# bi-graph/Emgraph

Measured on AMD Instinct MI355X. Metric: positive+negative triples scored/sec at k=200, eta=20; filtered ranks/sec, higher is better.
Workload: dtype f32; 1 GPU; C3: ComplEx k=200 (k_int=400) eta=20, synthetic |E|=1M |R|=1k, B=16384/GPU, NLL, SGD; B_per_gpu=16384, global_batch=16384, eta=20, k_int=400, k_int_per_gpu=400, n_ent=1000000, n_rel=1000, parallelism=single

## Files before the change

emgraph_amd/csrc/emg_score.hip:

```cpp
#include <math.h>
#include <string.h>

#include <atomic>

#include "emg_score_kernels.hpp"

namespace emg {

enum class Pass { Forward, Backward, Fused };

constexpr double kMallBytes = 256.0 * 1024 * 1024;
constexpr double kResidentBudget = 240e6;
static bool cache_policy_form(const GroupParams& P) {
    const int forced = sw_int(SW_CACHE_POLICY);
    if (forced == 0 || forced == 1) return forced == 1;
    const double n = (double)P.n_ent, row = 4.0 * (double)P.ld_ent;
    if (n < 2 || n * row <= kMallBytes) return false;
    const double N = (double)P.B * (2 + P.eta);
    const double l = log1p(-1.0 / n);
    const double distinct = n * -expm1(N * l), singles = N * exp((N - 1) * l);
    const double multi = distinct > singles ? distinct - singles : 0.0;
    const double contrib = 5.0 * (double)P.B + (P.fac.coef ? 0.0 : (N - singles));
    return (multi + contrib) * row <= kResidentBudget;
}

static std::atomic<int64_t> g_cache_policy_launches{0};

enum RidersGo : int32_t { RIDERS_NONE = 0, RIDERS_RIDE = 1, RIDERS_ALONE = 2 };
struct StepForm {
    Pass pass; int32_t model, n;
    int32_t W, shape;
    int32_t ip;
    bool wave_per_group, cache_policy, linked;
    int32_t riders;
    int32_t blocks;
};
static const int32_t kShape[8][2] = {{1, 16}, {1, 32}, {1, 64}, {2, 64}, {1, 64}, {2, 64}, {4, 64}, {8, 64}};
static int ladder(bool vec, int c, bool wave_per_group) {
    if (vec) return c <= 16 && !wave_per_group ? 0 : (c <= 32 && !wave_per_group ? 1 : (c <= kWaveChunks ? 2 : (c <= kMaxChunks ? 3 : -1)));
    return c <= 64 ? 4 : (c <= 128 ? 5 : (c <= 256 ? 6 : (c <= kColumnBlock ? 7 : -1)));
}

static int decide_step_form(Pass pass, int model, const GroupParams& P, bool have_riders, StepForm* out) {
    StepForm f{};
    f.pass = pass; f.model = model;
    const int n = f.n = step_columns(model, P.k_int);
    if (P.lr_hist && P.opt.opt == EMG_OPT_SGD) {
        EMG_REQUIRE(replay_rows(n, kMaxChunks, P.ld_ent, P.ent),
                    "emg_train_backward_ex: lr_hist needs 16-byte rows of at most %d chunks (per half for complex models)", kMaxChunks);
    } else if (P.lr_hist) {
        EMG_REQUIRE(replay_rows(n, kWaveChunks, P.ld_ent, P.ent) && aligned16(P.ent_state0) && aligned16(P.ent_state1) && !P.ctl,
                    "emg_train_backward_ex: lr_hist needs 16-byte rows of at most %d chunks (per half for complex models) and no device-side step record", kWaveChunks);
    }
    const bool cplx = (model == EMG_COMPLEX || model == EMG_HOLE);
    EMG_REQUIRE(model >= 0 && model <= EMG_HOLE, "unknown model id %d", model);
    EMG_REQUIRE(P.k_int > 0 && (!cplx || P.k_int % 2 == 0), "bad k_int %d for model %d", P.k_int, model);
    EMG_REQUIRE(P.ld_ent >= P.k_int && P.ld_rel >= P.k_int, "row stride smaller than k_int");
    EMG_REQUIRE(P.B >= 0 && P.eta >= 0, "negative sizes");
    if (P.B == 0) { *out = f; return EMG_OK; }
    EMG_REQUIRE(P.B * (int64_t)kThreads < ((int64_t)1 << 37), "batch too large");
    bool vec = (n % 4 == 0) && (P.ld_ent % 4 == 0) && (P.ld_rel % 4 == 0) && aligned16(P.ent) && aligned16(P.rel);
    if (pass != Pass::Forward) {
        vec = vec && (P.ldc % 4 == 0) && aligned16(P.contrib_ent) && aligned16(P.contrib_rel);
        if (P.single_ent)
            vec = vec && (!P.ent_state0 || aligned16(P.ent_state0)) && (!P.ent_state1 || aligned16(P.ent_state1));
    }
    f.W = vec ? 4 : 1;
    const bool sgd = P.opt.opt == EMG_OPT_SGD;
    if (pass != Pass::Forward && P.single_ent && sgd && P.opt.lp_lambda != 0.f && !vec)
        return fail(EMG_ENOSUP, "train backward: in-place updates fold an LP regulariser for 16-byte aligned rows only (k, or k per "
                                "half for complex models, a multiple of 4); pass single_ent = NULL");
    if (P.window && !(vec && pass == Pass::Fused && n / 4 <= kWaveChunks && P.single_ent && !sgd))
        return fail(EMG_ENOSUP, "train backward: inplace_window (a stateful optimizer's state rows travelling with the table rows) needs the "
                                "fused kernel on 16-byte aligned rows of at most %d chunks (per half for complex models)", kWaveChunks);
    if (pass == Pass::Forward || !P.single_ent) f.ip = IP_NONE;
    else if (sgd) f.ip = P.opt.lp_lambda == 0.f ? IP_SGD : (P.lr_hist ? IP_SGD_LP_LAG : IP_SGD_LP);
    else if (!P.window) f.ip = IP_STATE;
    else f.ip = P.lr_hist ? IP_WINDOW_LAG : ((P.opt.opt == EMG_OPT_ADAM || P.opt.opt == EMG_OPT_ADAM_LAZY) ? IP_WINDOW_2 : IP_WINDOW_1);
    f.riders = !have_riders ? RIDERS_NONE : ((pass == Pass::Fused && vec && n <= kColumnBlock) ? RIDERS_RIDE : RIDERS_ALONE);
    const int wide_env = sw_int(SW_WIDE_GROUPS);
    f.wave_per_group = f.ip >= IP_WINDOW_1 || (pass != Pass::Forward && (wide_env >= 0 ? wide_env != 0 : P.B <= 2048));
    f.blocks = 1; f.shape = ladder(vec, n / f.W, f.wave_per_group);
    if (f.shape < 0 && pass == Pass::Fused)
        return fail(EMG_ENOSUP, "fused score+loss+gradient: rows of k_int=%d are wider than the register-tiled kernel holds "
                                "(512 columns per half) — use emg_train_forward + emg_loss + emg_train_backward_ex(fused_loss = -1), "
                                "which splits wide rows into column blocks", P.k_int);
    if (f.shape < 0 && pass == Pass::Backward) {
        EMG_REQUIRE(model != EMG_TRANSE_L2 || (P.bw_scores_pos && (P.eta == 0 || P.bw_scores_neg)),
                    "train backward: TransE-L2 rows wider than 512 columns need bw_scores_pos / bw_scores_neg (the full norms)");
        f.blocks = (int32_t)cdiv(n, kColumnBlock);
        f.shape = ladder(vec, kColumnBlock / f.W, f.wave_per_group);
    }
    f.linked = pass == Pass::Fused && (P.link != EMG_LINK_LINEAR || P.edge_w);
    f.cache_policy = pass == Pass::Fused && f.shape == 2 && f.ip == IP_SGD && cache_policy_form(P);
    *out = f;
    return EMG_OK;
}

struct ShapeKernels { GroupKernel forward, backward[4], fused[2][3]; };
struct ModelKernels { ShapeKernels shape[8]; GroupKernel generic_forward; };
template <int M, int W, int NV, int LPG>
static constexpr ShapeKernels shape_kernels() {
    ShapeKernels s{train_forward_kernel<M, W, NV, LPG>,
                   {train_backward_kernel<M, W, NV, LPG, false, 0>, train_backward_kernel<M, W, NV, LPG, false, 1>, train_backward_kernel<M, W, NV, LPG, false, 2>, nullptr}, {}};
    if constexpr (W == 4) s.backward[3] = train_backward_kernel<M, W, NV, LPG, false, 3>;
    else s = {s.forward, {s.backward[0], s.backward[1], s.backward[2], nullptr},
              {{train_backward_kernel<M, W, NV, LPG, true, 0>, train_backward_kernel<M, W, NV, LPG, true, 1>, train_backward_kernel<M, W, NV, LPG, true, 2>},
               {train_backward_kernel<M, W, NV, LPG, true, 0, true>, train_backward_kernel<M, W, NV, LPG, true, 1, true>, train_backward_kernel<M, W, NV, LPG, true, 2, true>}}};
    return s;
}
template <int M>
static constexpr ModelKernels model_kernels() {
    return {{shape_kernels<M, 4, 1, 16>(), shape_kernels<M, 4, 1, 32>(), shape_kernels<M, 4, 1, 64>(), shape_kernels<M, 4, 2, 64>(),
             shape_kernels<M, 1, 1, 64>(), shape_kernels<M, 1, 2, 64>(), shape_kernels<M, 1, 4, 64>(), shape_kernels<M, 1, 8, 64>()}, train_forward_generic_kernel<M>};
}
static_assert(EMG_TRANSE_L1 == 0 && EMG_HOLE == 4, "the kernel tables are indexed by the model");
static const ModelKernels kModelKernels[5] = {model_kernels<0>(), model_kernels<1>(), model_kernels<2>(), model_kernels<3>(), model_kernels<4>()};
typedef FusedKernel (*FusedLookup)(int shape, int ip, bool cache_policy);
static const FusedLookup kFusedLookup[2][5] = {
    {fused_kernel<0, false>, fused_kernel<1, false>, fused_kernel<2, false>, fused_kernel<3, false>, fused_kernel<4, false>},
    {fused_kernel<0, true>, fused_kernel<1, true>, fused_kernel<2, true>, fused_kernel<3, true>, fused_kernel<4, true>}};
static GroupKernel group_kernel(const StepForm& f, int shape) {
    if (shape < 0) return kModelKernels[f.model].generic_forward;
    const ShapeKernels& s = kModelKernels[f.model].shape[shape];
    if (f.pass == Pass::Forward) return s.forward;
    if (f.pass == Pass::Backward) return f.ip <= IP_SGD_LP ? s.backward[f.ip] : nullptr;
    return f.ip <= IP_STATE ? s.fused[f.linked][f.ip] : nullptr;
}

static int launch_step(const StepForm& f, GroupParams& P, hipStream_t st, const Riders* riders_in, bool dry) {
    static const Riders no_riders{};
    const int rc = f.riders == RIDERS_ALONE && !dry ? launch_riders_alone(*riders_in, st) : EMG_OK;
    if (rc != EMG_OK) return rc;
    const Riders& riders = f.riders == RIDERS_RIDE && !dry ? *riders_in : no_riders;
    P.khalf = (f.model == EMG_COMPLEX || f.model == EMG_HOLE) ? f.n : 0;
    P.nchunks = f.n / f.W;
    for (int b = 0; b < f.blocks; ++b) {
        GroupParams Q = P;
        int shape = f.shape;
        if (f.blocks > 1) {
            const int c0 = b * kColumnBlock;
            Q.width = f.n - c0 < kColumnBlock ? f.n - c0 : kColumnBlock;
            Q.nchunks = Q.width / f.W;
            shape = ladder(f.W == 4, Q.nchunks, f.wave_per_group);
            Q.ent += c0; Q.rel += c0; Q.contrib_ent += c0; Q.contrib_rel += c0;
            if (Q.ent_rw) Q.ent_rw += c0;
            if (Q.ent_state0) Q.ent_state0 += c0;
            if (Q.ent_state1) Q.ent_state1 += c0;
        }
        const bool with_riders = f.pass == Pass::Fused && f.W == 4;
        const FusedKernel kf = with_riders ? kFusedLookup[f.linked][f.model](shape, f.ip, f.cache_policy) : nullptr;
        const GroupKernel kg = with_riders ? nullptr : group_kernel(f, shape);
        if (!kf && !kg)
            return fail(EMG_ENOSUP, "training step: no kernel for pass %d of model %d, %d-float chunks, shape %d, in-place form %d%s%s", (int)f.pass,
                        f.model, f.W, shape, f.ip, f.cache_policy ? ", cache policy" : "", f.linked ? ", linked" : "");
        if (dry) continue;
        const unsigned grid = (unsigned)cdiv(P.B, kThreads / (shape < 0 ? 64 : kShape[shape][1])) + riders.total;
        if (kf && f.cache_policy) g_cache_policy_launches.fetch_add(1);
        if (kf) hipLaunchKernelGGL(kf, dim3(grid), dim3(kThreads), 0, st, Q, riders);
        else hipLaunchKernelGGL(kg, dim3(grid), dim3(kThreads), 0, st, Q);
        EMG_LAUNCH_CHECK();
    }
    return EMG_OK;
}

static int run_group_pass(Pass pass, int model, GroupParams& P, hipStream_t st, const Riders* riders = nullptr, bool have_riders = false,
                          int32_t* form_out = nullptr) {
    StepForm f;
    int rc = decide_step_form(pass, model, P, have_riders, &f);
    if (rc == EMG_OK) rc = launch_step(f, P, st, riders, form_out != nullptr);
    if (rc != EMG_OK || !form_out) return rc;
    const int32_t fields[8] = {(int32_t)f.pass, f.model, f.W, f.shape < 0 ? 0 : kShape[f.shape][0], f.shape < 0 ? 64 : kShape[f.shape][1], f.ip,
                               (f.cache_policy ? 1 : 0) | (f.linked ? 2 : 0) | (f.riders << 2), f.blocks};
    memcpy(form_out, fields, sizeof(fields));
    return EMG_OK;
}
// ... 428 lines not shown
```

emgraph_amd/csrc/emg_score_kernels.hpp:

```cpp
#pragma once
#include "emg_group_kernels.hpp"

#pragma clang fp contract(off)

namespace emg {

template <int MODEL>
struct is_complex {
    static constexpr bool value = (MODEL == EMG_COMPLEX || MODEL == EMG_HOLE);
};

template <int MODEL, int W, int NV>
struct Row {
    static constexpr int E = W * NV;
    static constexpr int N = is_complex<MODEL>::value ? 2 * E : E;
    float x[N];
};

template <int MODEL, int W, int NV, int LPG, bool ZERO = true, bool NT = false>
__device__ __forceinline__ void load_row(Row<MODEL, W, NV>& r, const float* __restrict__ base, int lg, int nchunks,
                                         int khalf) {
    constexpr int E = W * NV;
    RowTile<W, NV> t;
    load_tile<W, NV, LPG, ZERO, NT>(t, base, lg, nchunks);
// ... 273 lines not shown
        }
    }
    if (P.tag_ent && lg == 0) P.tag_ent[row] = P.step;
}

template <int MODEL, int W, int NV, int LPG, int NS>
__device__ __forceinline__ void inplace_update_regs(const GroupParams& P, const OptParams& opt, int64_t row, const Row<MODEL, W, NV>& cur,
                                                    const Row<MODEL, W, NV>& grad, Row<MODEL, W, NV>& s0, Row<MODEL, W, NV>& s1, int lg) {
    static_assert(W == 4, "16-byte rows");
    constexpr int E = W * NV;
    constexpr int HALVES = is_complex<MODEL>::value ? 2 : 1;
    float* wrow = P.ent_rw + row * P.ld_ent;
    float* s0row = P.ent_state0 + row * P.ld_ent;
    float* s1row = NS == 2 ? P.ent_state1 + row * P.ld_ent : nullptr;
#pragma unroll
    for (int h = 0; h < HALVES; ++h) {
#pragma unroll
        for (int it = 0; it < NV; ++it) {
            const int c = lg + it * LPG;
            float wv[W];
#pragma unroll
            for (int w = 0; w < W; ++w) {
                const int e = h * E + it * W + w;
                wv[w] = cur.x[e];
                opt_update_elem(opt, wv[w], grad.x[e], &s0.x[e], NS == 2 ? &s1.x[e] : nullptr);
                __builtin_amdgcn_sched_barrier(0);
            }
            if (c < P.nchunks) {
                const int off = h * P.khalf + c * W;
                *reinterpret_cast<float4*>(wrow + off) = make_float4(wv[0], wv[1], wv[2], wv[3]);
                *reinterpret_cast<float4*>(s0row + off) = make_float4(s0.x[h * E + it * W], s0.x[h * E + it * W + 1], s0.x[h * E + it * W + 2], s0.x[h * E + it * W + 3]);
                if constexpr (NS == 2)
                    *reinterpret_cast<float4*>(s1row + off) = make_float4(s1.x[h * E + it * W], s1.x[h * E + it * W + 1], s1.x[h * E + it * W + 2], s1.x[h * E + it * W + 3]);
            }
        }
    }
    if (P.tag_ent && lg == 0) P.tag_ent[row] = P.step;
}

template <int MODEL, int W, int NV, int LPG>
__device__ __forceinline__ void replay_in_window(const GroupParams& P, const OptParams& opt0, int32_t from, float lrv, Row<MODEL, W, NV>& w,
                                                 Row<MODEL, W, NV>& m, Row<MODEL, W, NV>& v, int lg) {
    static_assert(LPG == 64, "the replay's step count is per wave");
    constexpr int E = W * NV;
    OptParams opt = opt0;
    const int n = P.upto - from;
    auto one_step = [&](float lr) {
        opt.lr = opt.lr_t = lr;
#pragma unroll
        for (int e = 0; e < Row<MODEL, W, NV>::N; ++e) {
            const bool on = lg + ((e % E) / W) * LPG < P.nchunks;
            float wv = w.x[e];
            adam_zero_grad_elem(opt, wv, m.x[e], v.x[e]);
            w.x[e] = on ? wv : w.x[e];
            __builtin_amdgcn_sched_barrier(0);
        }
    };
    const int n1 = n < 64 ? n : 64;
    for (int i = 0; i < n1; ++i) one_step(__int_as_float(__builtin_amdgcn_readlane(__float_as_int(lrv), i)));
    for (int i = 64; i < n; ++i) one_step(P.lr_hist[from + 1 + i]);
}

template <int MODEL, int W, int NV>
__device__ __forceinline__ void make_queries(const Row<MODEL, W, NV>& s, const Row<MODEL, W, NV>& p,
                                             const Row<MODEL, W, NV>& o, Row<MODEL, W, NV>& qo,
                                             Row<MODEL, W, NV>& qs) {
    constexpr int E = W * NV;
#pragma unroll
    for (int e = 0; e < E; ++e) {
        if constexpr (MODEL == EMG_TRANSE_L1 || MODEL == EMG_TRANSE_L2) {
            qo.x[e] = s.x[e] + p.x[e];
            qs.x[e] = o.x[e] - p.x[e];
        } else if constexpr (MODEL == EMG_DISTMULT) {
            qo.x[e] = p.x[e] * s.x[e];
            qs.x[e] = p.x[e] * o.x[e];
        } else {
            const float sr = s.x[e], si = s.x[E + e], pr = p.x[e], pi = p.x[E + e], orr = o.x[e], oi = o.x[E + e];
            qo.x[e] = fmaf(pr, sr, -(pi * si));   qo.x[E + e] = fmaf(pr, si, pi * sr);
            qs.x[e] = fmaf(pr, orr, pi * oi);     qs.x[E + e] = fmaf(pr, oi, -(pi * orr));
        }
    }
}

template <int MODEL, int W, int NV>
__device__ __forceinline__ float neg_partial(const Row<MODEL, W, NV>& q, const Row<MODEL, W, NV>& e) {
    float acc = 0.f;
#pragma unroll
    for (int i = 0; i < Row<MODEL, W, NV>::N; ++i) {
        if constexpr (MODEL == EMG_TRANSE_L1) acc += fabsf(q.x[i] - e.x[i]);
        else if constexpr (MODEL == EMG_TRANSE_L2) { const float d = q.x[i] - e.x[i]; acc = fmaf(d, d, acc); }
        else acc = fmaf(q.x[i], e.x[i], acc);
    }
    return acc;
}

template <int MODEL, int W, int NV, bool OBJ>
__device__ __forceinline__ void neg_grads(const Row<MODEL, W, NV>& q, const Row<MODEL, W, NV>& e, float gi,
                                          Row<MODEL, W, NV>& row, Row<MODEL, W, NV>& acc) {
#pragma unroll
    for (int i = 0; i < Row<MODEL, W, NV>::N; ++i) {
        if constexpr (MODEL == EMG_TRANSE_L1 || MODEL == EMG_TRANSE_L2) {
            const float d = OBJ ? q.x[i] - e.x[i] : e.x[i] - q.x[i];
            const float t = (MODEL == EMG_TRANSE_L1) ? gi * sgnf(d) : gi * d;
            row.x[i] = OBJ ? t : -t;
            acc.x[i] += t;
        } else {
            row.x[i] = gi * q.x[i];
            acc.x[i] = fmaf(gi, e.x[i], acc.x[i]);
        }
    }
}

template <int MODEL, int W, int NV>
__device__ __forceinline__ void finish_grads(const Row<MODEL, W, NV>& s, const Row<MODEL, W, NV>& p,
                                             const Row<MODEL, W, NV>& o, const Row<MODEL, W, NV>& Ao,
                                             const Row<MODEL, W, NV>& As, float gp_i, Row<MODEL, W, NV>& gs,
                                             Row<MODEL, W, NV>& gp, Row<MODEL, W, NV>& go) {
    constexpr int E = W * NV;
#pragma unroll
    for (int e = 0; e < E; ++e) {
        if constexpr (MODEL == EMG_TRANSE_L1 || MODEL == EMG_TRANSE_L2) {
            const float d = (s.x[e] + p.x[e]) - o.x[e];
            const float tp = (MODEL == EMG_TRANSE_L1) ? gp_i * sgnf(d) : gp_i * d;
            gs.x[e] = -Ao.x[e] - tp;
            gp.x[e] = -Ao.x[e] - As.x[e] - tp;
            go.x[e] = As.x[e] + tp;
        } else if constexpr (MODEL == EMG_DISTMULT) {
            const float bo = fmaf(gp_i, o.x[e], Ao.x[e]);
            const float bs = fmaf(gp_i, s.x[e], As.x[e]);
            gs.x[e] = p.x[e] * bo;
            go.x[e] = p.x[e] * bs;
            gp.x[e] = fmaf(s.x[e], bo, As.x[e] * o.x[e]);
        } else {
            const float sr = s.x[e], si = s.x[E + e], pr = p.x[e], pi = p.x[E + e], orr = o.x[e], oi = o.x[E + e];
            const float br = fmaf(gp_i, orr, Ao.x[e]), bi = fmaf(gp_i, oi, Ao.x[E + e]);
            const float ar = fmaf(gp_i, sr, As.x[e]), ai = fmaf(gp_i, si, As.x[E + e]);
            gs.x[e] = fmaf(pr, br, pi * bi);          gs.x[E + e] = fmaf(pr, bi, -(pi * br));
            go.x[e] = fmaf(pr, ar, -(pi * ai));       go.x[E + e] = fmaf(pr, ai, pi * ar);
            gp.x[e] = fmaf(sr, br, si * bi) + fmaf(As.x[e], orr, As.x[E + e] * oi);
            gp.x[E + e] = fmaf(sr, bi, -(si * br)) + fmaf(As.x[e], oi, -(As.x[E + e] * orr));
        }
    }
}

constexpr int kBwU = 4;
constexpr int kBwMinWaves = 1;

typedef float emg_f4 __attribute__((ext_vector_type(4)));
__device__ __forceinline__ emg_f4 vm_load16_async(const float* p) {
    emg_f4 v;
    asm volatile("global_load_dwordx4 %0, %1, off" : "=v"(v) : "v"(p) : "memory");
    return v;
}
__device__ __forceinline__ float vm_load4_async(const float* p) {
    float v;
    asm volatile("global_load_dword %0, %1, off" : "=v"(v) : "v"(p) : "memory");
    return v;
}
__device__ __forceinline__ void vm_landed(emg_f4& a) { asm volatile("" : "+v"(a) : : "memory"); }
__device__ __forceinline__ void vm_landed(float& a) { asm volatile("" : "+v"(a) : : "memory"); }
template <int N> __device__ __forceinline__ void vm_wait_only() { asm volatile("s_waitcnt vmcnt(%0)" : : "n"(N) : "memory"); }

template <int MODEL, int W, int NV, bool FUSED, int IP>
struct keep_rows {
    static constexpr bool value = W == 4 && NV == 1 && ip_traits<IP>::n_state != 2 &&
                                  (!is_complex<MODEL>::value || (FUSED && (IP == 1 || IP == 2)));
};
template <int MODEL, int W, int NV, int LPG, bool FUSED, int IP, bool CP = false, bool LINKED = false>
__device__ __forceinline__ void train_backward_body(const GroupParams& P0, unsigned bx) {
    static_assert(!LINKED || FUSED, "the link acts where the loss is taken: the fused forms");
    static_assert(!CP || (IP == 1 && W == 4), "the cache-policy form is plain SGD in place on 16-byte rows");
    constexpr bool STREAM_C = !CP;
    using R = Row<MODEL, W, NV>;
    GroupParams P = P0;
    if (P0.ctl) {
        P.B = P0.ctl->B; P.pos = P0.pos + 3 * P0.ctl->start; P.step = P0.ctl->step;
        if (P0.edge_w) P.edge_w = P0.edge_w + P0.ctl->start;
        P.opt.lr = P0.ctl->hyper_ent[0]; P.opt.lr_t = P0.ctl->hyper_ent[5];
    }
    const int lg = threadIdx.x % LPG;
    int64_t g = ((int64_t)bx * kThreads + threadIdx.x) / LPG;
    if ((int64_t)bx * (kThreads / LPG) >= P.B) return;
    const bool active = g < P.B;
    if (!active) g = P.B - 1;
    const int64_t B = P.B;
    constexpr bool kBilinear = !(MODEL == EMG_TRANSE_L1 || MODEL == EMG_TRANSE_L2);

    const int32_t s = P.pos[3 * g + 0], p = P.pos[3 * g + 1], o = P.pos[3 * g + 2];
    const float* srow = P.ent + (int64_t)s * P.ld_ent;
    const float* prow = P.rel + (int64_t)p * P.ld_rel;
    const float* orow = P.ent + (int64_t)o * P.ld_ent;
    const int first = (threadIdx.x & 63) / LPG * LPG;
    using IT = ip_traits<IP>;
    constexpr int NS = IT::n_state;
    static_assert(!IT::window_state || (W == 4 && LPG == 64 && FUSED), "IP 4 / 5 / 6: fused kernels of 16-byte rows, a wave per group");
    static_assert(!IT::lp_replay || (W == 4 && LPG == 64 && FUSED), "IP 7: fused kernels of 16-byte rows, a wave per group");
    int my_code = 0, my_flag = 0, my_pos = 0, my_flag_so = 0;
    int my_tag = 0;
    auto gather = [&](int c0) {
        const int j = c0 + lg;
        my_code = j < P.eta ? P.codes[(int64_t)j * B + g] : 0;
        if (kBilinear && P.fac.coef) my_pos = j < P.eta ? (int)P.fac.pos_of_slot[(int64_t)j * B + g] : 0;
        if constexpr (IP != 0) my_flag = j < P.eta ? (int)P.single_ent[2 * B + (int64_t)j * B + g] : 0;
        if constexpr (IT::replay || IT::lp_replay) my_tag = (j < P.eta && my_flag) ? P.tag_ent[my_code & 0x7fffffff] : P.upto;
    };
    gather(0);
    float lr_lane = 0.f;
    if constexpr (IT::lp_replay) lr_lane = P.lr_hist[max(P.upto - lg, 0)];
    if constexpr (IT::so_inplace) { if (lg < 2) my_flag_so = P.single_ent[(int64_t)lg * B + g]; }
    OptParams wopt = P.opt;
    if constexpr (NS == 2) wopt.opt = EMG_OPT_ADAM;
    R qo, qs, Ao, As;
    float pos_nrm = 0.f, pos_score = 0.f, gpos = 0.f, loss_acc = 0.f, lp_acc = 0.f;
    constexpr bool KEEP = keep_rows<MODEL, W, NV, FUSED, IP>::value;
    R ks, kp, ko;
    constexpr bool SOP = IT::window_state;
    float* stash = nullptr;
    int fso0 = 0, fso1 = 0;
    int tso0 = 0, tso1 = 0;
    if constexpr (SOP) {
        __shared__ float so_stash_mem[kThreads / 64][2 * (1 + NS)][R::N][64];
        stash = &so_stash_mem[threadIdx.x >> 6][0][0][0];
    }
    auto park = [&](int slot, const R& r) {
#pragma unroll
        for (int e = 0; e < R::N; ++e) stash[(slot * R::N + e) * 64 + lg] = r.x[e];
    };
    auto unpark = [&](int slot, R& r) {
#pragma unroll
        for (int e = 0; e < R::N; ++e) r.x[e] = stash[(slot * R::N + e) * 64 + lg];
    };
    {
        R rs, rp, ro;
        load_row<MODEL, W, NV, LPG, true, CP>(rs, srow, lg, P.nchunks, P.khalf);
        load_row<MODEL, W, NV, LPG>(rp, prow, lg, P.nchunks, P.khalf);
        load_row<MODEL, W, NV, LPG, true, CP>(ro, orow, lg, P.nchunks, P.khalf);
        if constexpr (SOP) {
            int my_tag_so = 0;
            if constexpr (IT::replay) { my_tag_so = P.upto; if (lg < 2) my_tag_so = P.tag_ent[lg == 0 ? s : o]; }
            fso0 = group_lane_value<LPG>(my_flag_so, first, 0); fso1 = group_lane_value<LPG>(my_flag_so, first, 1);
            R ms, vs, mo, vo;
            load_row<MODEL, W, NV, LPG, false>(ms, fso0 ? P.ent_state0 + (int64_t)s * P.ld_ent : srow, lg, P.nchunks, P.khalf);
            load_row<MODEL, W, NV, LPG, false>(mo, fso1 ? P.ent_state0 + (int64_t)o * P.ld_ent : orow, lg, P.nchunks, P.khalf);
            if constexpr (NS == 2) {
                load_row<MODEL, W, NV, LPG, false>(vs, fso0 ? P.ent_state1 + (int64_t)s * P.ld_ent : srow, lg, P.nchunks, P.khalf);
                load_row<MODEL, W, NV, LPG, false>(vo, fso1 ? P.ent_state1 + (int64_t)o * P.ld_ent : orow, lg, P.nchunks, P.khalf);
            }
            if constexpr (IT::replay) {
                const int ts = group_lane_value<LPG>(my_tag_so, first, 0), to = group_lane_value<LPG>(my_tag_so, first, 1);
                const float lrs = P.lr_hist[min(ts + 1 + lg, P.upto)], lro = P.lr_hist[min(to + 1 + lg, P.upto)];
                if (fso0 && ts > 0 && ts < P.upto) replay_in_window<MODEL, W, NV, LPG>(P, wopt, ts, lrs, rs, ms, vs, lg);
                if (fso1 && to > 0 && to < P.upto) replay_in_window<MODEL, W, NV, LPG>(P, wopt, to, lro, ro, mo, vo, lg);
            }
            park(0, rs); park(1, ms); park(1 + NS, ro); park(2 + NS, mo);
            if constexpr (NS == 2) { park(2, vs); park(5, vo); }
        }
        if constexpr (IT::lp_replay) {
            int my_tag_so = P.upto;
            if (lg < 2) my_tag_so = P.tag_ent[lg == 0 ? s : o];
            fso0 = group_lane_value<LPG>(my_flag_so, first, 0); fso1 = group_lane_value<LPG>(my_flag_so, first, 1);
            tso0 = fso0 ? __builtin_amdgcn_readfirstlane(group_lane_value<LPG>(my_tag_so, first, 0)) : P.upto;
            tso1 = fso1 ? __builtin_amdgcn_readfirstlane(group_lane_value<LPG>(my_tag_so, first, 1)) : P.upto;
            float counted = 0.f;
            if (tso0 < P.upto) lp_replay_row<MODEL, W, NV, LPG>(P, tso0, lr_lane, rs, lg, counted);
            if (tso1 < P.upto) lp_replay_row<MODEL, W, NV, LPG>(P, tso1, lr_lane, ro, lg, counted);
            if (active) lp_acc += counted;
        }
        make_queries<MODEL, W, NV>(rs, rp, ro, qo, qs);
        if constexpr (KEEP) { ks = rs; kp = rp; ko = ro; }
        if constexpr (FUSED || MODEL == EMG_TRANSE_L2) {
            if (MODEL == EMG_TRANSE_L2 && P.bw_scores_pos) {
                pos_nrm = -P.bw_scores_pos[g];
            } else {
                const float sum = group_sum<LPG>(partial_score<MODEL, W, NV>(rs, rp, ro));
                pos_score = finalize_score<MODEL>(sum, P.scale, 0);
                if constexpr (MODEL == EMG_TRANSE_L2) pos_nrm = sqrtf(sum);
            }
        }
    }
#pragma unroll
    for (int e = 0; e < R::N; ++e) Ao.x[e] = As.x[e] = 0.f;
    PosTerms pos_terms{0.f, 0.f};
    constexpr bool linked = LINKED;
    float* link_park = nullptr;
    if constexpr (LINKED) {
        __shared__ float link_park_mem[3][kThreads];
        link_park = &link_park_mem[0][threadIdx.x];
    }
    if constexpr (FUSED) {
        if (P.scores_pos && active && lg == 0) P.scores_pos[g] = pos_score;
        if constexpr (linked) {
            float w_pos = 1.f, w_neg = 1.f;
            if (P.edge_w) {
                const float w = P.edge_w[g];
                w_pos = focuse_weight_pos(P.sw, w);
                w_neg = focuse_weight_neg(P.sw, w);
            }
            const LinkTerms lt = link_apply(P.link, w_pos, pos_score);
            pos_score = lt.s;
            link_park[0] = w_neg;
            link_park[kThreads] = lt.d;
        }
        pos_terms = local_loss_pos(P.fused_loss, pos_score);
    } else {
        gpos = P.g_pos[g];
    }

    constexpr int kWinBudget = 48;
    constexpr int U = !IT::window_state ? kBwU : (R::N * (1 + NS) * 4 <= kWinBudget ? 4 : (R::N * (1 + NS) * 3 <= kWinBudget ? 3 : 2));
    int chunk0 = 0, chunk1 = min(P.eta, LPG);
    auto code_of = [&](int j) -> int32_t { return group_lane_value<LPG>(my_code, first, j - chunk0); };
    auto flag_of = [&](int j) -> int {
        if constexpr (IP == 0) return 0;
        return group_lane_value<LPG>(my_flag, first, j - chunk0);
    };
    auto flag_so = [&](int which) -> int {
        if constexpr (IP == 0) return 0;
        return group_lane_value<LPG>(my_flag_so, first, which);
    };
    constexpr int PIECES_S = NV * (is_complex<MODEL>::value ? 2 : 1);
    constexpr int LPS = PIECES_S * (1 + NS) + (IT::replay ? 1 : 0);
    static_assert(!IT::window_state || (U - 1) * LPS <= 63, "vmcnt is a 6-bit counter");
    R st0[IT::window_state ? U : 1], st1[NS == 2 ? U : 1];
    int32_t tg[IT::replay ? U : 1];
    float lrv[IT::replay ? U : 1];
    emg_f4 aw[IT::window_state ? U : 1][IT::window_state ? PIECES_S : 1], a0[IT::window_state ? U : 1][IT::window_state ? PIECES_S : 1],
           a1[NS == 2 ? U : 1][NS == 2 ? PIECES_S : 1];
    constexpr bool kZeroAtUse = !kBilinear;
    auto zero_tail = [&](R& r) {
#pragma unroll
        for (int e = 0; e < R::N; ++e) r.x[e] = (lg + ((e % (W * NV)) / W) * LPG < P.nchunks) ? r.x[e] : 0.f;
    };
    auto issue_slot = [&](int u, int jn, int32_t repl) {
        if constexpr (IT::window_state) {
            const bool f = flag_of(jn) != 0;
            const float* wb = P.ent + (int64_t)repl * P.ld_ent;
            const float* b0 = f ? P.ent_state0 + (int64_t)repl * P.ld_ent : wb;
            const float* b1 = (NS == 2 && f) ? P.ent_state1 + (int64_t)repl * P.ld_ent : wb;
#pragma unroll
            for (int h = 0; h < (is_complex<MODEL>::value ? 2 : 1); ++h)
#pragma unroll
                for (int it = 0; it < NV; ++it) {
                    const int off = h * P.khalf + 4 * min(lg + it * LPG, P.nchunks - 1);
                    aw[u][h * NV + it] = vm_load16_async(wb + off);
                    a0[u][h * NV + it] = vm_load16_async(b0 + off);
                    if constexpr (NS == 2) a1[u][h * NV + it] = vm_load16_async(b1 + off);
                }
            if constexpr (IT::replay) {
                tg[u] = group_lane_value<LPG>(my_tag, first, jn - chunk0);
                lrv[u] = vm_load4_async(P.lr_hist + min(tg[u] + 1 + lg, P.upto));
            }
        }
    };
    auto unpack = [&](const emg_f4 (&src)[IT::window_state ? PIECES_S : 1], R& r, bool zero_tail) {
#pragma unroll
        for (int q = 0; q < PIECES_S; ++q) {
            const bool on = !zero_tail || lg + (q % NV) * LPG < P.nchunks;
            r.x[4 * q + 0] = on ? src[q].x : 0.f; r.x[4 * q + 1] = on ? src[q].y : 0.f;
            r.x[4 * q + 2] = on ? src[q].z : 0.f; r.x[4 * q + 3] = on ? src[q].w : 0.f;
        }
    };
    auto take_slot = [&](int u, R& w_row) {
        if constexpr (IT::window_state) {
            vm_wait_only<(U - 1) * LPS>();
#pragma unroll
            for (int q = 0; q < PIECES_S; ++q) { vm_landed(aw[u][q]); vm_landed(a0[u][q]); if constexpr (NS == 2) vm_landed(a1[u][q]); }
            if constexpr (IT::replay) vm_landed(lrv[u]);
            unpack(aw[u], w_row, !kBilinear);
            unpack(a0[u], st0[u], false);
            if constexpr (NS == 2) unpack(a1[u], st1[u], false);
        }
    };
    auto fetch = [&](int j0, int32_t (&code)[U], R (&re)[U]) {
#pragma unroll
        for (int u = 0; u < U; ++u) code[u] = code_of(min(j0 + u, chunk1 - 1));
#pragma unroll
        for (int u = 0; u < U; ++u) {
            const int32_t repl = code[u] & 0x7fffffff;
            if constexpr (IT::window_state) issue_slot(u, min(j0 + u, chunk1 - 1), repl);
            else load_row<MODEL, W, NV, LPG, false, CP>(re[u], P.ent + (int64_t)repl * P.ld_ent, lg, P.nchunks, P.khalf);
        }
    };
    int32_t code[U];
    float gj[U];
    R re[U];
    for (; chunk0 < P.eta; chunk0 += LPG) {
    chunk1 = min(P.eta, chunk0 + LPG);
    if (chunk0 > 0) gather(chunk0);
    fetch(chunk0, code, re);
    if constexpr (!FUSED) {
#pragma unroll
        for (int u = 0; u < U; ++u) gj[u] = P.g_neg[(int64_t)min(chunk0 + u, chunk1 - 1) * B + g];
    }
    for (int j0 = chunk0; j0 < chunk1; j0 += U) {
#pragma unroll
        for (int u = 0; u < U; ++u) {
            const int j = j0 + u;
            if (j >= chunk1) break;
            const bool keep_s = code[u] < 0;
            const int32_t repl = code[u] & 0x7fffffff;
            if constexpr (IT::window_state) take_slot(u, re[u]);
            if constexpr (kZeroAtUse && !IT::window_state) zero_tail(re[u]);
            if constexpr (IT::replay) {
                if (flag_of(j) && tg[u] > 0 && tg[u] < P.upto) replay_in_window<MODEL, W, NV, LPG>(P, wopt, tg[u], lrv[u], re[u], st0[u], st1[u], lg);
            }
            if constexpr (IT::lp_replay) {
                const int from = __builtin_amdgcn_readfirstlane(group_lane_value<LPG>(my_tag, first, j - chunk0));
                float counted = 0.f;
                if (from < P.upto) lp_replay_row<MODEL, W, NV, LPG>(P, from, lr_lane, re[u], lg, counted);
                if (active) lp_acc += counted;
            }
            float nrm = 0.f;
            if constexpr (FUSED || MODEL == EMG_TRANSE_L2) {
                if (MODEL == EMG_TRANSE_L2 && P.bw_scores_neg) {
                    nrm = -P.bw_scores_neg[(int64_t)j * B + g];
                } else {
                    float part;
                    if (keep_s) part = neg_partial<MODEL, W, NV>(qo, re[u]);
                    else part = neg_partial<MODEL, W, NV>(qs, re[u]);
                    const float sum = group_sum<LPG>(part);
                    if constexpr (MODEL == EMG_TRANSE_L2) nrm = sqrtf(sum);
                    if constexpr (FUSED) {
                        const float neg = finalize_score<MODEL>(sum, P.scale, 0);
                        float eff = neg;
                        if constexpr (linked) {
                            const LinkTerms lt = link_apply(P.link, link_park[0], neg);
                            link_park[2 * kThreads] = lt.d;
                            eff = lt.s;
                        }
                        gj[u] = local_loss_neg(P.fused_loss, pos_score, pos_terms, eff, P.margin, loss_acc, gpos);
                        if constexpr (linked) gj[u] *= link_park[2 * kThreads];
                        if (P.scores_neg && active && lg == 0) P.scores_neg[(int64_t)j * B + g] = neg;
                    }
                }
            }
            const float gi = inner_coef<MODEL>(gj[u], nrm, P.scale);
            R row;
            if (keep_s) neg_grads<MODEL, W, NV, true>(qo, re[u], gi, row, Ao);
            else neg_grads<MODEL, W, NV, false>(qs, re[u], gi, row, As);
            if (active) {
                const int64_t slot = 2 * B + (int64_t)j * B + g;
                if (IP != 0 && flag_of(j)) {
                    if constexpr (IT::window_state) inplace_update_regs<MODEL, W, NV, LPG, NS>(P, wopt, repl, re[u], row, st0[u], st1[NS == 2 ? u : 0], lg);
                    else inplace_update<MODEL, W, NV, LPG, IT::chunkwise, CP>(P, repl, re[u], row, lg, lp_acc);
                }
                else if (kBilinear && P.fac.coef) {
                    const int at = group_lane_value<LPG>(my_pos, first, j - chunk0);
                    if (lg == 0) P.fac.coef[at] = gi;
                }
                else store_row<MODEL, W, NV, LPG, STREAM_C>(row, P.contrib_ent + slot * P.ldc, lg, P.nchunks, P.khalf);
            }
            const int jn = min(j + U, chunk1 - 1);
            code[u] = code_of(jn);
            if constexpr (IT::window_state) issue_slot(u, jn, code[u] & 0x7fffffff);
            else load_row<MODEL, W, NV, LPG, false, CP>(re[u], P.ent + (int64_t)(code[u] & 0x7fffffff) * P.ld_ent, lg, P.nchunks, P.khalf);
            if constexpr (!FUSED) gj[u] = P.g_neg[(int64_t)jn * B + g];
        }
    }
    if constexpr (IT::window_state) {
        vm_wait_only<0>();
#pragma unroll
        for (int u = 0; u < U; ++u) {
#pragma unroll
            for (int q = 0; q < PIECES_S; ++q) { vm_landed(aw[u][q]); vm_landed(a0[u][q]); if constexpr (NS == 2) vm_landed(a1[u][q]); }
            if constexpr (IT::replay) vm_landed(lrv[u]);
        }
    }
    }
    if (kBilinear && P.fac.coef && active) {
        store_row<MODEL, W, NV, LPG, STREAM_C>(qo, P.contrib_ent + (2 * B + g) * P.ldc, lg, P.nchunks, P.khalf);
        store_row<MODEL, W, NV, LPG, STREAM_C>(qs, P.contrib_ent + (3 * B + g) * P.ldc, lg, P.nchunks, P.khalf);
    }
    int32_t es = s, ep = p, eo = o;
    int64_t eg = g;
    if constexpr (IT::window_state) asm volatile("" : "+v"(es), "+v"(ep), "+v"(eo), "+v"(eg));
    const float* srow_e = P.ent + (int64_t)es * P.ld_ent;
    const float* prow_e = P.rel + (int64_t)ep * P.ld_rel;
    const float* orow_e = P.ent + (int64_t)eo * P.ld_ent;
    if (active) {
        R rs, rp, ro, gs, gp, go;
        if constexpr (KEEP) {
            rs = ks; rp = kp; ro = ko;
        } else {
            load_row<MODEL, W, NV, LPG>(rs, srow_e, lg, P.nchunks, P.khalf);
            load_row<MODEL, W, NV, LPG>(rp, prow_e, lg, P.nchunks, P.khalf);
            load_row<MODEL, W, NV, LPG>(ro, orow_e, lg, P.nchunks, P.khalf);
        }
        if constexpr (IT::replay) {
            if (fso0) unpark(0, rs);
            if (fso1) unpark(1 + NS, ro);
        }
        if constexpr (IT::lp_replay && !KEEP) {
            float uncounted = 0.f;
            if (tso0 < P.upto) lp_replay_row<MODEL, W, NV, LPG>(P, tso0, lr_lane, rs, lg, uncounted);
            if (tso1 < P.upto) lp_replay_row<MODEL, W, NV, LPG>(P, tso1, lr_lane, ro, lg, uncounted);
        }
        if constexpr (linked) gpos *= link_park[kThreads];
        finish_grads<MODEL, W, NV>(rs, rp, ro, Ao, As, inner_coef<MODEL>(gpos, pos_nrm, P.scale), gs, gp, go);
        store_row<MODEL, W, NV, LPG>(gp, P.contrib_rel + eg * P.ldc, lg, P.nchunks, P.khalf);
        if constexpr (SOP) {
            if (fso0) { R ms, vs; unpark(1, ms); if constexpr (NS == 2) unpark(2, vs); inplace_update_regs<MODEL, W, NV, LPG, NS>(P, wopt, es, rs, gs, ms, vs, lg); }
            else store_row<MODEL, W, NV, LPG>(gs, P.contrib_ent + eg * P.ldc, lg, P.nchunks, P.khalf);
            if (fso1) { R mo, vo; unpark(2 + NS, mo); if constexpr (NS == 2) unpark(5, vo); inplace_update_regs<MODEL, W, NV, LPG, NS>(P, wopt, eo, ro, go, mo, vo, lg); }
            else store_row<MODEL, W, NV, LPG>(go, P.contrib_ent + (B + eg) * P.ldc, lg, P.nchunks, P.khalf);
        } else {
            if (IT::so_inplace && flag_so(0)) inplace_update<MODEL, W, NV, LPG, IT::chunkwise, CP>(P, es, rs, gs, lg, lp_acc);
            else store_row<MODEL, W, NV, LPG, STREAM_C>(gs, P.contrib_ent + eg * P.ldc, lg, P.nchunks, P.khalf);
            if (IT::so_inplace && flag_so(1)) inplace_update<MODEL, W, NV, LPG, IT::chunkwise, CP>(P, eo, ro, go, lg, lp_acc);
            else store_row<MODEL, W, NV, LPG, STREAM_C>(go, P.contrib_ent + (B + eg) * P.ldc, lg, P.nchunks, P.khalf);
        }
    }
    if constexpr (IP == 3 || IP == 7) block_add_double(P.lp_accum, lp_acc);
    if constexpr (FUSED) {
        double v = (active && lg == 0) ? (double)loss_acc : 0.0;
#pragma unroll
        for (int off = 32; off >= 1; off >>= 1) v += __shfl_xor(v, off, 64);
        __shared__ double part[kThreads / 64];
        if ((threadIdx.x & 63) == 0) part[threadIdx.x >> 6] = v;
        __syncthreads();
        if (threadIdx.x == 0) {
            double t = 0.0;
#pragma unroll
            for (int w = 0; w < kThreads / 64; ++w) t += part[w];
            if (t != 0.0) atomicAdd(P.loss_accum + (bx & P.loss_mask), t);
        }
    }
}

template <int MODEL, int W, int NV, int LPG, bool FUSED, int IP, bool LINKED = false>
__global__ __launch_bounds__(kThreads, kBwMinWaves) void train_backward_kernel(const GroupParams P) {
    train_backward_body<MODEL, W, NV, LPG, FUSED, IP, false, LINKED>(P, blockIdx.x);
}
#ifdef EMG_TRACE
static __device__ unsigned long long emg_trace_fused_buf[4 * 65536];
#endif
constexpr int kWindowMinWaves = 3;
template <int MODEL, int W, int NV, int LPG, int IP, bool CP = false, bool LINKED = false>
__global__ __launch_bounds__(kThreads, (ip_traits<IP>::window_state ? kWindowMinWaves : kBwMinWaves)) void train_fused_riders_kernel(const GroupParams P, const Riders riders) {
    unsigned bx;
    if (run_riders(riders, &bx)) return;
#ifdef EMG_TRACE
    const unsigned tw = (bx * kThreads + threadIdx.x) >> 6;
    if ((threadIdx.x & 63) == 0 && tw < 65536) emg_trace_fused_buf[4 * tw] = wall_clock64();
#endif
    train_backward_body<MODEL, W, NV, LPG, true, IP, CP, LINKED>(P, bx);
#ifdef EMG_TRACE
    if ((threadIdx.x & 63) == 0 && tw < 65536) emg_trace_fused_buf[4 * tw + 1] = wall_clock64();
#endif
}

static __global__ void build_dest_kernel(const int32_t* __restrict__ pos, int64_t B, int eta, const int32_t* __restrict__ codes,
                                  int32_t* __restrict__ dest_ent, int32_t* __restrict__ dest_rel) {
    const int64_t t = (int64_t)blockIdx.x * blockDim.x + threadIdx.x;
    if (t < B) {
        dest_ent[t] = pos[3 * t + 0];
        dest_ent[B + t] = pos[3 * t + 2];
        dest_rel[t] = pos[3 * t + 1];
    }
    if (t < (int64_t)eta * B) dest_ent[2 * B + t] = codes[t] & 0x7fffffff;
}

template <int MODEL>
__device__ __forceinline__ float strided_partial(const float* __restrict__ a, const float* __restrict__ p,
                                                 const float* __restrict__ b, int khalf, int n, int lane) {
    float acc = 0.f;
    for (int c = lane; c < n; c += 64) {
        if constexpr (MODEL == EMG_TRANSE_L1) {
            acc += fabsf((a[c] + p[c]) - b[c]);
        } else if constexpr (MODEL == EMG_TRANSE_L2) {
            const float d = (a[c] + p[c]) - b[c];
            acc = fmaf(d, d, acc);
        } else if constexpr (MODEL == EMG_DISTMULT) {
            acc = fmaf(a[c] * p[c], b[c], acc);
        } else {
            const float sr = a[c], si = a[khalf + c], pr = p[c], pi = p[khalf + c], orr = b[c], oi = b[khalf + c];
            acc = fmaf(pr * sr, orr, acc);
            acc = fmaf(pr * si, oi, acc);
            acc = fmaf(pi * sr, oi, acc);
            acc = fmaf(-(pi * si), orr, acc);
        }
    }
    return acc;
}

template <int MODEL>
__global__ __launch_bounds__(kThreads) void train_forward_generic_kernel(const GroupParams P) {
    const int lane = threadIdx.x & 63;
    int64_t g = ((int64_t)blockIdx.x * kThreads + threadIdx.x) / 64;
    const bool active = g < P.B;
    if (!active) g = P.B - 1;
    const int n = is_complex<MODEL>::value ? P.khalf : P.k_int;
    const float* rs = P.ent + (int64_t)P.pos[3 * g + 0] * P.ld_ent;
    const float* rp = P.rel + (int64_t)P.pos[3 * g + 1] * P.ld_rel;
    const float* ro = P.ent + (int64_t)P.pos[3 * g + 2] * P.ld_ent;
    float sum = group_sum<64>(strided_partial<MODEL>(rs, rp, ro, P.khalf, n, lane));
    if (active && lane == 0) P.scores_pos[g] = finalize_score<MODEL>(sum, P.scale, P.flags);
    for (int j = 0; j < P.eta; ++j) {
        const int32_t code = P.codes[(int64_t)j * P.B + g];
        const float* re = P.ent + (int64_t)(code & 0x7fffffff) * P.ld_ent;
        const bool keep_s = code < 0;
        sum = group_sum<64>(strided_partial<MODEL>(keep_s ? rs : re, rp, keep_s ? re : ro, P.khalf, n, lane));
        if (active && lane == 0) P.scores_neg[(int64_t)j * P.B + g] = finalize_score<MODEL>(sum, P.scale, P.flags);
    }
}


__device__ __forceinline__ float wave_sum_f(float v) {
#pragma unroll
    for (int off = 32; off >= 1; off >>= 1) v += __shfl_xor(v, off, 64);
    return v;
}
__device__ __forceinline__ float wave_max_f(float v) {
#pragma unroll
    for (int off = 32; off >= 1; off >>= 1) v = fmaxf(v, __shfl_xor(v, off, 64));
    return v;
}
__device__ __forceinline__ float transe_p_norm(const float* a, const float* p, const float* b, int k_int, float ord, int lane, float* ties) {
    const bool mx = isinf(ord);
    float acc = 0.f;
    for (int c = lane; c < k_int; c += 64) {
        const float d = fabsf((a[c] + p[c]) - b[c]);
        acc = mx ? fmaxf(acc, d) : acc + powf(d, ord);
    }
    if (!mx) return powf(wave_sum_f(acc), 1.0f / ord);
    acc = wave_max_f(acc);
    if (ties) {
        float cnt = 0.f;
        for (int c = lane; c < k_int; c += 64) cnt += fabsf((a[c] + p[c]) - b[c]) == acc ? 1.f : 0.f;
        *ties = wave_sum_f(cnt);
    }
    return acc;
}

enum InPlace : int32_t {
    IP_NONE = 0, IP_SGD = 1, IP_STATE = 2, IP_SGD_LP = 3,
    IP_WINDOW_1 = 4, IP_WINDOW_2 = 5, IP_WINDOW_LAG = 6, IP_SGD_LP_LAG = 7
};
typedef void (*GroupKernel)(const GroupParams);
typedef void (*FusedKernel)(const GroupParams, const Riders);
template <int MODEL, bool LINKED> FusedKernel fused_kernel(int shape, int ip, bool cache_policy);

}
```

Baseline: 1.120 billion triples scored/s.

## Pick per-row nontemporal loads for negatives in cache-policy backward form

In the cache-policy backward form, negative-entity rows are now fetched with async dwordx4 loads through the window slot machinery, which adds explicit vmcnt waits. Each load chooses at runtime between a nontemporal and a normal cache policy based on a per-negative flag, so rows that are touched once do not evict reused rows from the last-level cache. The relation gradient store now follows the same streaming policy as the entity stores. The residency estimate that decides whether to use this form now counts relation contributions separately from entity contributions. The CP form also now requires a full wave per group.

```diff
diff --git a/emgraph_amd/csrc/emg_score.hip b/emgraph_amd/csrc/emg_score.hip
--- a/emgraph_amd/csrc/emg_score.hip
+++ b/emgraph_amd/csrc/emg_score.hip
@@ -20,8 +20,9 @@
     const double l = log1p(-1.0 / n);
     const double distinct = n * -expm1(N * l), singles = N * exp((N - 1) * l);
     const double multi = distinct > singles ? distinct - singles : 0.0;
-    const double contrib = 5.0 * (double)P.B + (P.fac.coef ? 0.0 : (N - singles));
-    return (multi + contrib) * row <= kResidentBudget;
+    const double contrib = 4.0 * (double)P.B + (P.fac.coef ? 0.0 : (N - singles));
+    const double contrib_rel = (double)P.B * 4.0 * (double)P.ld_rel;
+    return (multi + contrib) * row + contrib_rel <= kResidentBudget;
 }
 
 static std::atomic<int64_t> g_cache_policy_launches{0};
diff --git a/emgraph_amd/csrc/emg_score_kernels.hpp b/emgraph_amd/csrc/emg_score_kernels.hpp
--- a/emgraph_amd/csrc/emg_score_kernels.hpp
+++ b/emgraph_amd/csrc/emg_score_kernels.hpp
@@ -449,6 +449,12 @@
     asm volatile("global_load_dwordx4 %0, %1, off" : "=v"(v) : "v"(p) : "memory");
     return v;
 }
+__device__ __forceinline__ emg_f4 vm_load16_async_pick(const float* p, int nt) {
+    emg_f4 v;
+    asm volatile("s_cmp_eq_u32 %2, 0\n\ts_cbranch_scc1 1f\n\tglobal_load_dwordx4 %0, %1, off nt\n\ts_branch 2f\n1:\n\tglobal_load_dwordx4 %0, %1, off\n2:"
+                 : "=v"(v) : "v"(p), "s"(nt) : "scc", "memory");
+    return v;
+}
 __device__ __forceinline__ float vm_load4_async(const float* p) {
     float v;
     asm volatile("global_load_dword %0, %1, off" : "=v"(v) : "v"(p) : "memory");
@@ -466,7 +472,7 @@
 template <int MODEL, int W, int NV, int LPG, bool FUSED, int IP, bool CP = false, bool LINKED = false>
 __device__ __forceinline__ void train_backward_body(const GroupParams& P0, unsigned bx) {
     static_assert(!LINKED || FUSED, "the link acts where the loss is taken: the fused forms");
-    static_assert(!CP || (IP == 1 && W == 4), "the cache-policy form is plain SGD in place on 16-byte rows");
+    static_assert(!CP || (IP == 1 && W == 4 && LPG == 64), "the cache-policy form is plain SGD in place on 16-byte rows, a wave per group");
     constexpr bool STREAM_C = !CP;
     using R = Row<MODEL, W, NV>;
     GroupParams P = P0;
@@ -617,11 +623,12 @@
     };
     constexpr int PIECES_S = NV * (is_complex<MODEL>::value ? 2 : 1);
     constexpr int LPS = PIECES_S * (1 + NS) + (IT::replay ? 1 : 0);
-    static_assert(!IT::window_state || (U - 1) * LPS <= 63, "vmcnt is a 6-bit counter");
+    static_assert(!(IT::window_state || CP) || (U - 1) * LPS <= 63, "vmcnt is a 6-bit counter");
     R st0[IT::window_state ? U : 1], st1[NS == 2 ? U : 1];
     int32_t tg[IT::replay ? U : 1];
     float lrv[IT::replay ? U : 1];
-    emg_f4 aw[IT::window_state ? U : 1][IT::window_state ? PIECES_S : 1], a0[IT::window_state ? U : 1][IT::window_state ? PIECES_S : 1],
+    constexpr bool ASYNC = IT::window_state || CP;
+    emg_f4 aw[ASYNC ? U : 1][ASYNC ? PIECES_S : 1], a0[IT::window_state ? U : 1][IT::window_state ? PIECES_S : 1],
            a1[NS == 2 ? U : 1][NS == 2 ? PIECES_S : 1];
     constexpr bool kZeroAtUse = !kBilinear;
     auto zero_tail = [&](R& r) {
@@ -647,9 +654,17 @@
                 tg[u] = group_lane_value<LPG>(my_tag, first, jn - chunk0);
                 lrv[u] = vm_load4_async(P.lr_hist + min(tg[u] + 1 + lg, P.upto));
             }
-        }
-    };
-    auto unpack = [&](const emg_f4 (&src)[IT::window_state ? PIECES_S : 1], R& r, bool zero_tail) {
+        } else if constexpr (CP) {
+            const int nt = uniform_if_wave<LPG>(flag_of(jn));
+            const float* wb = P.ent + (int64_t)repl * P.ld_ent;
+#pragma unroll
+            for (int h = 0; h < (is_complex<MODEL>::value ? 2 : 1); ++h)
+#pragma unroll
+                for (int it = 0; it < NV; ++it)
+                    aw[u][h * NV + it] = vm_load16_async_pick(wb + h * P.khalf + 4 * min(lg + it * LPG, P.nchunks - 1), nt);
+        }
+    };
+    auto unpack = [&](const emg_f4 (&src)[ASYNC ? PIECES_S : 1], R& r, bool zero_tail) {
 #pragma unroll
         for (int q = 0; q < PIECES_S; ++q) {
             const bool on = !zero_tail || lg + (q % NV) * LPG < P.nchunks;
@@ -666,6 +681,11 @@
             unpack(aw[u], w_row, !kBilinear);
             unpack(a0[u], st0[u], false);
             if constexpr (NS == 2) unpack(a1[u], st1[u], false);
+        } else if constexpr (CP) {
+            vm_wait_only<(U - 1) * LPS>();
+#pragma unroll
+            for (int q = 0; q < PIECES_S; ++q) vm_landed(aw[u][q]);
+            unpack(aw[u], w_row, !kBilinear);
         }
     };
     auto fetch = [&](int j0, int32_t (&code)[U], R (&re)[U]) {
@@ -675,7 +695,8 @@
         for (int u = 0; u < U; ++u) {
             const int32_t repl = code[u] & 0x7fffffff;
             if constexpr (IT::window_state) issue_slot(u, min(j0 + u, chunk1 - 1), repl);
-            else load_row<MODEL, W, NV, LPG, false, CP>(re[u], P.ent + (int64_t)repl * P.ld_ent, lg, P.nchunks, P.khalf);
+            else if constexpr (CP) issue_slot(u, min(j0 + u, chunk1 - 1), repl);
+            else load_row<MODEL, W, NV, LPG, false>(re[u], P.ent + (int64_t)repl * P.ld_ent, lg, P.nchunks, P.khalf);
         }
     };
     int32_t code[U];
@@ -696,8 +717,8 @@
             if (j >= chunk1) break;
             const bool keep_s = code[u] < 0;
             const int32_t repl = code[u] & 0x7fffffff;
-            if constexpr (IT::window_state) take_slot(u, re[u]);
-            if constexpr (kZeroAtUse && !IT::window_state) zero_tail(re[u]);
+            if constexpr (ASYNC) take_slot(u, re[u]);
+            if constexpr (kZeroAtUse && !ASYNC) zero_tail(re[u]);
             if constexpr (IT::replay) {
                 if (flag_of(j) && tg[u] > 0 && tg[u] < P.upto) replay_in_window<MODEL, W, NV, LPG>(P, wopt, tg[u], lrv[u], re[u], st0[u], st1[u], lg);
             }
@@ -750,7 +771,8 @@
             const int jn = min(j + U, chunk1 - 1);
             code[u] = code_of(jn);
             if constexpr (IT::window_state) issue_slot(u, jn, code[u] & 0x7fffffff);
-            else load_row<MODEL, W, NV, LPG, false, CP>(re[u], P.ent + (int64_t)(code[u] & 0x7fffffff) * P.ld_ent, lg, P.nchunks, P.khalf);
+            else if constexpr (CP) issue_slot(u, jn, code[u] & 0x7fffffff);
+            else load_row<MODEL, W, NV, LPG, false>(re[u], P.ent + (int64_t)(code[u] & 0x7fffffff) * P.ld_ent, lg, P.nchunks, P.khalf);
             if constexpr (!FUSED) gj[u] = P.g_neg[(int64_t)jn * B + g];
         }
     }
@@ -762,6 +784,12 @@
             for (int q = 0; q < PIECES_S; ++q) { vm_landed(aw[u][q]); vm_landed(a0[u][q]); if constexpr (NS == 2) vm_landed(a1[u][q]); }
             if constexpr (IT::replay) vm_landed(lrv[u]);
         }
+    } else if constexpr (CP) {
+        vm_wait_only<0>();
+#pragma unroll
+        for (int u = 0; u < U; ++u)
+#pragma unroll
+            for (int q = 0; q < PIECES_S; ++q) vm_landed(aw[u][q]);
     }
     }
     if (kBilinear && P.fac.coef && active) {
@@ -794,7 +822,7 @@
         }
         if constexpr (linked) gpos *= link_park[kThreads];
         finish_grads<MODEL, W, NV>(rs, rp, ro, Ao, As, inner_coef<MODEL>(gpos, pos_nrm, P.scale), gs, gp, go);
-        store_row<MODEL, W, NV, LPG>(gp, P.contrib_rel + eg * P.ldc, lg, P.nchunks, P.khalf);
+        store_row<MODEL, W, NV, LPG, STREAM_C>(gp, P.contrib_rel + eg * P.ldc, lg, P.nchunks, P.khalf);
         if constexpr (SOP) {
             if (fso0) { R ms, vs; unpark(1, ms); if constexpr (NS == 2) unpark(2, vs); inplace_update_regs<MODEL, W, NV, LPG, NS>(P, wopt, es, rs, gs, ms, vs, lg); }
             else store_row<MODEL, W, NV, LPG>(gs, P.contrib_ent + eg * P.ldc, lg, P.nchunks, P.khalf);
```

Result: faster. 1.149 billion triples scored/s (median of 6 runs) (+2.6%).
